# alibaba/TePDist

Hardware: AMD Instinct MI355X
Metric: tokens/sec (higher is better)
Workload: dtype bf16; 1 GPU; model=gpt2-345m, global_batch=64, seq_len=1024, parallelism=auto-planned-graph:dp1tp1pp1mesh[]micro1

## Files before the change

### tepdist_amd/ops/csrc/attention.hip

```cpp

#include <algorithm>
#include <stdexcept>

#include "common.h"
#include "kernels.h"
#include "lds_frag.h"

namespace tepdist {

namespace {

constexpr int NT = 256;
constexpr int QB = 128;
constexpr int KB = 64;

constexpr float kLog2e = 1.4426950408889634f;
DEV_INLINE float fast_exp(float x) {
  return __builtin_amdgcn_exp2f(x * kLog2e);
}

#define BAR_LDS()                                        \
  do {                                                   \
    asm volatile("s_waitcnt lgkmcnt(0)" ::: "memory");   \
    __builtin_amdgcn_s_barrier();                        \
  } while (0)

DEV_INLINE float warp16_max(float v) {
#pragma unroll
  for (int d = 1; d < 16; d <<= 1) v = fmaxf(v, __shfl_xor(v, d, 64));
  return v;
}

DEV_INLINE float warp16_sum(float v) {
#pragma unroll
  for (int d = 1; d < 16; d <<= 1) v += __shfl_xor(v, d, 64);
  return v;
}


constexpr int NTF = 512;
constexpr int QBF = 512;

template <int NQ>
DEV_INLINE int pair_row0(int q0, int wave, int hp) {
  return NQ == 4 ? q0 + 32 * (hp ? 15 - wave : wave) : q0 + 32 * wave;
}

template <int D, int NQ = (D == 64 ? 4 : 2)>
__launch_bounds__(NTF) __global__
void flash_fwd_kernel(const bf16_t* __restrict__ Q,
                      const bf16_t* __restrict__ K,
                      const bf16_t* __restrict__ V, bf16_t* __restrict__ O,
                      float* __restrict__ LSE, int S, int H, float scale,
                      bool causal, int64_t q_bs, int64_t q_hs, int64_t q_rs,
                      int64_t o_bs, int64_t o_hs, int64_t o_rs) {
  constexpr int DK = D / 32;
  constexpr int DF = D / 16;
  const int bh = blockIdx.y;
  const int b = bh / H, h = bh % H;
  const int q0 = blockIdx.x * (128 * NQ);
  const int wave = __builtin_amdgcn_readfirstlane(threadIdx.x >> 6);
  const int lane = threadIdx.x & 63;
  const int g = lane >> 4;

  const bf16_t* qp = Q + (int64_t)b * q_bs + (int64_t)h * q_hs;
  const bf16_t* kp = K + (int64_t)b * q_bs + (int64_t)h * q_hs;
  const bf16_t* vp = V + (int64_t)b * q_bs + (int64_t)h * q_hs;
  bf16_t* op = O + (int64_t)b * o_bs + (int64_t)h * o_hs;

  __shared__ __attribute__((aligned(16))) bf16_t smem[2 * 2 * KB * D];
  const int BUFSZ = 2 * KB * D;

  bf16x8 qf[NQ][DK];
#pragma unroll
  for (int nf = 0; nf < NQ; ++nf)
#pragma unroll
    for (int kk = 0; kk < DK; ++kk) {
      const int row = pair_row0<NQ>(q0, wave, nf >> 1) + (nf & 1) * 16 +
                      (lane & 15);
      bf16x8 v8 = {};
      if (row < S)
        v8 = *reinterpret_cast<const bf16x8*>(
            qp + (int64_t)row * q_rs + kk * 32 + 8 * g);
      qf[nf][kk] = v8;
    }

  const float sl2 = scale * kLog2e;
  f32x4 acc_o[DF][NQ] = {};
  float m_r[NQ], l_r[NQ];
#pragma unroll
  for (int i = 0; i < NQ; ++i) {
    m_r[i] = -3.0e38f;
    l_r[i] = 0.f;
  }

  constexpr int KUN = KB * D / 8 / NTF;
  bf16x8 krg[KUN], vrg[KUN];

  auto stage_load = [&](int kv0) {
#pragma unroll
    for (int u = 0; u < KUN; ++u) {
      const int idx = threadIdx.x + u * NTF;
      const int row = idx / (D / 8);
      const int c = (idx % (D / 8)) * 8;
      bf16x8 k8 = {}, v8 = {};
      if (kv0 + row < S) {
        k8 = *reinterpret_cast<const bf16x8*>(
            kp + (int64_t)(kv0 + row) * q_rs + c);
        v8 = *reinterpret_cast<const bf16x8*>(
            vp + (int64_t)(kv0 + row) * q_rs + c);
      }
      krg[u] = k8;
      vrg[u] = v8;
    }
  };
  auto stage_write = [&](int buf) {
    bf16_t* sK = smem + buf * BUFSZ;
    bf16_t* sV = sK + KB * D;
#pragma unroll
    for (int u = 0; u < KUN; ++u) {
      const int idx = threadIdx.x + u * NTF;
      const int row = idx / (D / 8);
      const int c = (idx % (D / 8)) * 8;
      *reinterpret_cast<bf16x8*>(sK + loff<D>(row, c)) = krg[u];
      *reinterpret_cast<bf16x8*>(sV + loff<D>(row, c)) = vrg[u];
    }
  };

  const int kv_end = causal ? min(S, q0 + 128 * NQ) : S;
  stage_load(0);
  stage_write(0);
  __syncthreads();
  int t = 0;
  for (int kv0 = 0; kv0 < kv_end; kv0 += KB, ++t) {
    const bf16_t* sK = smem + (t & 1) * BUFSZ;
    const bf16_t* sV = sK + KB * D;
    if (kv0 + KB < kv_end) stage_load(kv0 + KB);

    if (!causal || kv0 <= pair_row0<NQ>(q0, wave, NQ / 2 - 1) + 31) {
#pragma unroll
      for (int hp = 0; hp < NQ / 2; ++hp) {
        const int pq0 = pair_row0<NQ>(q0, wave, hp);
        if (causal && kv0 > pq0 + 31) continue;
        f32x4 st[4][2] = {};
        __builtin_amdgcn_s_setprio(1);
#pragma unroll
        for (int kk = 0; kk < DK; ++kk)
#pragma unroll
          for (int mi = 0; mi < 4; ++mi) {
            const bf16x8 kf = *reinterpret_cast<const bf16x8*>(
                sK + loff<D>((lane & 15) + 16 * mi, 8 * g + 32 * kk));
#pragma unroll
            for (int nf = 0; nf < 2; ++nf)
              st[mi][nf] = __builtin_amdgcn_mfma_f32_16x16x32_bf16(
                  kf, qf[2 * hp + nf][kk], st[mi][nf], 0, 0, 0);
          }
        __builtin_amdgcn_s_setprio(0);
        const bool inner = kv0 + KB <= pq0 && kv0 + KB <= S &&
                           pq0 + 32 <= S;
#pragma unroll
        for (int nf = 0; nf < 2; ++nf) {
          const int nfg = 2 * hp + nf;
          const int qg = pq0 + nf * 16 + (lane & 15);
          float tmax = -3.0e38f;
          if (inner) {
#pragma unroll
            for (int mi = 0; mi < 4; ++mi)
#pragma unroll
              for (int e = 0; e < 4; ++e)
                tmax = fmaxf(tmax, st[mi][nf][e]);
          } else {
#pragma unroll
            for (int mi = 0; mi < 4; ++mi)
#pragma unroll
              for (int e = 0; e < 4; ++e) {
                const int kg = kv0 + mi * 16 + 4 * g + e;
                const bool masked = (causal && kg > qg) || kg >= S ||
                                    qg >= S;
                const float sv = masked ? -3.0e38f : st[mi][nf][e];
                st[mi][nf][e] = sv;
                tmax = fmaxf(tmax, sv);
              }
          }
          tmax = fmaxf(tmax, __shfl_xor(tmax, 16, 64));
          tmax = fmaxf(tmax, __shfl_xor(tmax, 32, 64));
          const float mn = fmaxf(m_r[nfg], tmax * scale);
          const float alpha = fast_exp(m_r[nfg] - mn);
          m_r[nfg] = mn;
          const float nm2 = -mn * kLog2e;
          float rs = 0.f;
#pragma unroll
          for (int mi = 0; mi < 4; ++mi)
#pragma unroll
            for (int e = 0; e < 4; ++e) {
              const float p = __builtin_amdgcn_exp2f(
                  __builtin_fmaf(st[mi][nf][e], sl2, nm2));
              st[mi][nf][e] = p;
              rs += p;
            }
          rs += __shfl_xor(rs, 16, 64);
          rs += __shfl_xor(rs, 32, 64);
          l_r[nfg] = l_r[nfg] * alpha + rs;
#pragma unroll
          for (int df = 0; df < DF; ++df)
#pragma unroll
            for (int e = 0; e < 4; ++e) acc_o[df][nfg][e] *= alpha;
        }
        __builtin_amdgcn_s_setprio(1);
#pragma unroll
        for (int c = 0; c < KB / 32; ++c) {
          bf16x8 pb[2];
#pragma unroll
          for (int nf = 0; nf < 2; ++nf)
#pragma unroll
            for (int e = 0; e < 4; ++e) {
              pb[nf][e] = f2bf(st[2 * c][nf][e]);
              pb[nf][e + 4] = f2bf(st[2 * c + 1][nf][e]);
            }
#pragma unroll
          for (int df = 0; df < DF; ++df) {
            const bf16x8 vfr = tr_frag<D>(sV, c, df, lane);
#pragma unroll
            for (int nf = 0; nf < 2; ++nf)
              acc_o[df][2 * hp + nf] = __builtin_amdgcn_mfma_f32_16x16x32_bf16(
                  vfr, pb[nf], acc_o[df][2 * hp + nf], 0, 0, 0);
          }
        }
        __builtin_amdgcn_s_setprio(0);
      }
    }
    if (kv0 + KB < kv_end) stage_write((t + 1) & 1);
    BAR_LDS();
  }

#pragma unroll
  for (int nf = 0; nf < NQ; ++nf) {
    const int qg = pair_row0<NQ>(q0, wave, nf >> 1) + (nf & 1) * 16 +
                   (lane & 15);
    if (qg >= S) continue;
    const float lv = l_r[nf];
    const float inv = (lv > 0.f) ? 1.0f / lv : 0.f;
    if (g == 0)
      LSE[(int64_t)bh * S + qg] =
          (lv > 0.f) ? m_r[nf] + __logf(lv) : -3.0e38f;
#pragma unroll
    for (int df = 0; df < DF; ++df)
#pragma unroll
      for (int e = 0; e < 4; ++e)
        op[(int64_t)qg * o_rs + 16 * df + 4 * g + e] =
            f2bf(acc_o[df][nf][e] * inv);
  }
}

}

void attention_fwd_bf16(const void* q, const void* k, const void* v, void* o,
                        float* lse, int B, int H, int S, int D, float scale,
                        bool causal, int64_t q_bs, int64_t q_hs, int64_t q_rs,
                        int64_t o_bs, int64_t o_hs, int64_t o_rs,
                        hipStream_t stream) {
  dim3 block(NTF);
#define FWD_D(DD)                                                        \
  do {                                                                   \
    dim3 grid((S + (DD == 64 ? QBF : 256) - 1) / (DD == 64 ? QBF : 256), \
              B * H);                                                    \
    hipLaunchKernelGGL(flash_fwd_kernel<DD>, grid, block, 0, stream,     \
                       static_cast<const bf16_t*>(q),                    \
                       static_cast<const bf16_t*>(k),                    \
                       static_cast<const bf16_t*>(v),                    \
                       static_cast<bf16_t*>(o), lse, S, H, scale,        \
                       causal, q_bs, q_hs, q_rs, o_bs, o_hs, o_rs);      \
  } while (0)
  if (D == 64) FWD_D(64);
  else if (D == 128) FWD_D(128);
  else throw std::runtime_error("flash fwd: head dim must be 64 or 128");
#undef FWD_D
}

namespace {


template <int D>
__launch_bounds__(NT) __global__
void flash_bwd_delta_kernel(const bf16_t* __restrict__ dO,
                            const bf16_t* __restrict__ O,
                            float* __restrict__ delta, int64_t rows) {
  const int lane = threadIdx.x & 63;
  const int wid = threadIdx.x >> 6;
  const int64_t nw = (int64_t)gridDim.x * (NT / WAVE);
  for (int64_t r = (int64_t)blockIdx.x * (NT / WAVE) + wid; r < rows;
       r += nw) {
    float s = 0.f;
    for (int c = lane * 8; c < D; c += WAVE * 8) {
      const bf16x8 a = *reinterpret_cast<const bf16x8*>(dO + r * D + c);
      const bf16x8 b = *reinterpret_cast<const bf16x8*>(O + r * D + c);
#pragma unroll
      for (int e = 0; e < 8; ++e) s += bf2f(a[e]) * bf2f(b[e]);
    }
    s = wave_allreduce_sum(s);
    if (lane == 0) delta[r] = s;
  }
}

constexpr int NTA = 512;

template <int D, int KBA = (D == 64 ? 256 : 128)>
__launch_bounds__(NTA) __global__
void flash_bwd_kv_kernel(const bf16_t* __restrict__ Q,
                         const bf16_t* __restrict__ K,
                         const bf16_t* __restrict__ V,
                         const bf16_t* __restrict__ dO,
                         const float* __restrict__ LSE,
                         const float* __restrict__ DELTA,
                         bf16_t* __restrict__ dK, bf16_t* __restrict__ dV,
                         int S, int H, float scale, bool causal,
                         int64_t q_bs, int64_t q_hs, int64_t q_rs,
                         int64_t o_bs, int64_t o_hs, int64_t o_rs) {
  constexpr int DK = D / 32;
  constexpr int DF = D / 16;
  constexpr int QT = 64;
  constexpr int NSL = KBA / 128;
  const int bh = blockIdx.y;
  const int b = bh / H, h = bh % H;
  const int kv0 = blockIdx.x * KBA;
  const int wave = __builtin_amdgcn_readfirstlane(threadIdx.x >> 6);
  const int lane = threadIdx.x & 63;
  const int g = lane >> 4;

  const int64_t qoff = (int64_t)b * q_bs + (int64_t)h * q_hs;
  const int64_t ooff = (int64_t)b * o_bs + (int64_t)h * o_hs;
  const bf16_t* qp = Q + qoff;
  const bf16_t* kp = K + qoff;
  const bf16_t* vp = V + qoff;
  const bf16_t* dop = dO + ooff;

  __shared__ __attribute__((aligned(16))) bf16_t
      smem[KBA * D * 2 + QT * D * 2];
  bf16_t* sKb = smem;
  bf16_t* sVb = sKb + KBA * D;
  bf16_t* sQ = sVb + KBA * D;
  bf16_t* sdO = sQ + QT * D;
  __shared__ __attribute__((aligned(16))) float sNL2[QT], sDELTA[QT];
  const float sl2 = scale * kLog2e;

  {
    constexpr int UN = KBA * D / 8 / NTA;
#pragma unroll
    for (int u = 0; u < UN; ++u) {
      const int idx = threadIdx.x + u * NTA;
      const int row = idx / (D / 8);
      const int c = (idx % (D / 8)) * 8;
      bf16x8 kv8 = {}, vv8 = {};
      if (kv0 + row < S) {
        kv8 = *reinterpret_cast<const bf16x8*>(
            kp + (int64_t)(kv0 + row) * q_rs + c);
        vv8 = *reinterpret_cast<const bf16x8*>(
            vp + (int64_t)(kv0 + row) * q_rs + c);
      }
      *reinterpret_cast<bf16x8*>(sKb + loff<D>(row, c)) = kv8;
      *reinterpret_cast<bf16x8*>(sVb + loff<D>(row, c)) = vv8;
    }
  }
  __syncthreads();

  f32x4 acc_dkT[NSL][DF] = {};
  f32x4 acc_dvT[NSL][DF] = {};

  constexpr int QUN = QT * D / 8 / NTA;
  bf16x8 qn[QUN], don[QUN];
  float lse2[QT / NTA + 1], dl2[QT / NTA + 1];

  auto tile_load = [&](int q0) {
#pragma unroll
    for (int u = 0; u < QUN; ++u) {
      const int idx = threadIdx.x + u * NTA;
      const int row = idx / (D / 8);
      const int c = (idx % (D / 8)) * 8;
      bf16x8 a = {}, b2 = {};
      if (q0 + row < S) {
        a = *reinterpret_cast<const bf16x8*>(
            qp + (int64_t)(q0 + row) * q_rs + c);
        b2 = *reinterpret_cast<const bf16x8*>(
            dop + (int64_t)(q0 + row) * o_rs + c);
      }
      qn[u] = a;
      don[u] = b2;
    }
    for (int i = threadIdx.x, s2 = 0; i < QT; i += NTA, ++s2) {
      const int qg = q0 + i;
      const float l = (qg < S) ? LSE[(int64_t)bh * S + qg] : -3.0e38f;
      lse2[s2] = (l > -1.0e38f) ? -l * kLog2e : -3.0e38f;
      dl2[s2] = (qg < S) ? DELTA[(int64_t)bh * S + qg] : 0.f;
    }
  };
  auto tile_write = [&]() {
#pragma unroll
    for (int u = 0; u < QUN; ++u) {
      const int idx = threadIdx.x + u * NTA;
      const int row = idx / (D / 8);
      const int c = (idx % (D / 8)) * 8;
      *reinterpret_cast<bf16x8*>(sQ + loff<D>(row, c)) = qn[u];
      *reinterpret_cast<bf16x8*>(sdO + loff<D>(row, c)) = don[u];
    }
    for (int i = threadIdx.x, s2 = 0; i < QT; i += NTA, ++s2) {
      sNL2[i] = lse2[s2];
      sDELTA[i] = dl2[s2];
    }
  };

  const int q_start = causal ? (kv0 / QT) * QT : 0;
  tile_load(q_start);
  tile_write();
  __syncthreads();
  for (int q0 = q_start; q0 < S; q0 += QT) {
    if (q0 + QT < S) tile_load(q0 + QT);

#pragma unroll
    for (int sl = 0; sl < NSL; ++sl) {
      if (causal && kv0 + sl * 128 + wave * 16 > q0 + QT - 1) continue;
      f32x4 st[4] = {};
      f32x4 dpt[4] = {};
#pragma unroll
      for (int kk = 0; kk < DK; ++kk) {
        const bf16x8 kfr = *reinterpret_cast<const bf16x8*>(
            sKb + loff<D>(sl * 128 + wave * 16 + (lane & 15),
                          8 * g + 32 * kk));
        const bf16x8 vfr = *reinterpret_cast<const bf16x8*>(
            sVb + loff<D>(sl * 128 + wave * 16 + (lane & 15),
                          8 * g + 32 * kk));
#pragma unroll
        for (int mi = 0; mi < 4; ++mi) {
          const bf16x8 qa = *reinterpret_cast<const bf16x8*>(
              sQ + loff<D>(16 * mi + (lane & 15), 8 * g + 32 * kk));
          st[mi] = __builtin_amdgcn_mfma_f32_16x16x32_bf16(qa, kfr,
                                                           st[mi], 0, 0, 0);
          const bf16x8 da = *reinterpret_cast<const bf16x8*>(
              sdO + loff<D>(16 * mi + (lane & 15), 8 * g + 32 * kk));
          dpt[mi] = __builtin_amdgcn_mfma_f32_16x16x32_bf16(
              da, vfr, dpt[mi], 0, 0, 0);
        }
      }

      const int kvb = kv0 + sl * 128;
      const int kvg = kvb + wave * 16 + (lane & 15);
      const bool winner = (!causal || kvb + wave * 16 + 15 < q0) &&
                          q0 + QT <= S && kvb + 128 <= S;
      if (winner) {
        f32x4 nl2v[4], dlv[4];
#pragma unroll
        for (int mi = 0; mi < 4; ++mi) {
          nl2v[mi] = *reinterpret_cast<const f32x4*>(sNL2 + 16 * mi + 4 * g);
          dlv[mi] = *reinterpret_cast<const f32x4*>(sDELTA + 16 * mi + 4 * g);
        }
#pragma unroll
        for (int mi = 0; mi < 4; ++mi)
#pragma unroll
          for (int e = 0; e < 4; ++e) {
            const float pt = __builtin_amdgcn_exp2f(
                __builtin_fmaf(st[mi][e], sl2, nl2v[mi][e]));
            st[mi][e] = pt;
            dpt[mi][e] = pt * (dpt[mi][e] - dlv[mi][e]);
          }
      } else {
#pragma unroll
        for (int mi = 0; mi < 4; ++mi)
#pragma unroll
          for (int e = 0; e < 4; ++e) {
            const int qrow = 16 * mi + 4 * g + e;
            const int qg = q0 + qrow;
            const float nl2 = sNL2[qrow];
            const float dl = sDELTA[qrow];
            const bool valid = qg < S && kvg < S && (!causal || kvg <= qg) &&
                               nl2 > -1.0e38f;
            const float arg =
                valid ? __builtin_fmaf(st[mi][e], sl2, nl2) : -3.0e38f;
            const float pt = __builtin_amdgcn_exp2f(arg);
            st[mi][e] = pt;
            dpt[mi][e] = pt * (dpt[mi][e] - dl);
          }
      }

      __builtin_amdgcn_s_setprio(1);
#pragma unroll
      for (int c = 0; c < QT / 32; ++c) {
        bf16x8 pb, db;
#pragma unroll
        for (int e = 0; e < 4; ++e) {
          pb[e] = f2bf(st[2 * c][e]);
          pb[e + 4] = f2bf(st[2 * c + 1][e]);
          db[e] = f2bf(dpt[2 * c][e]);
          db[e + 4] = f2bf(dpt[2 * c + 1][e]);
        }
#pragma unroll
        for (int df = 0; df < DF; ++df) {
          const bf16x8 afr = tr_frag<D>(sdO, c, df, lane);
          const bf16x8 qfr = tr_frag<D>(sQ, c, df, lane);
          acc_dvT[sl][df] = __builtin_amdgcn_mfma_f32_16x16x32_bf16(
              afr, pb, acc_dvT[sl][df], 0, 0, 0);
          acc_dkT[sl][df] = __builtin_amdgcn_mfma_f32_16x16x32_bf16(
              qfr, db, acc_dkT[sl][df], 0, 0, 0);
        }
      }
      __builtin_amdgcn_s_setprio(0);
    }
    BAR_LDS();
    if (q0 + QT < S) {
      tile_write();
      BAR_LDS();
    }
  }

#pragma unroll
  for (int sl = 0; sl < NSL; ++sl) {
    const int kvg = kv0 + sl * 128 + wave * 16 + (lane & 15);
    if (kvg < S) {
#pragma unroll
      for (int df = 0; df < DF; ++df) {
        bf16x4 kv4, vv4;
#pragma unroll
        for (int e = 0; e < 4; ++e) {
          kv4[e] = f2bf(acc_dkT[sl][df][e] * scale);
          vv4[e] = f2bf(acc_dvT[sl][df][e]);
        }
        const int64_t off = qoff + (int64_t)kvg * q_rs + 16 * df + 4 * g;
        *reinterpret_cast<bf16x4*>(dK + off) = kv4;
        *reinterpret_cast<bf16x4*>(dV + off) = vv4;
      }
    }
  }
}

constexpr int NTB = 512;
constexpr int QBB = 256;

template <int D, int NQ = (D == 64 ? 4 : 2)>
__launch_bounds__(NTB) __global__
void flash_bwd_dq_kernel(const bf16_t* __restrict__ Q,
                         const bf16_t* __restrict__ K,
                         const bf16_t* __restrict__ V,
                         const bf16_t* __restrict__ dO,
                         const float* __restrict__ LSE,
                         const float* __restrict__ DELTA,
                         bf16_t* __restrict__ dQ, int S, int H, float scale,
                         bool causal, int64_t q_bs, int64_t q_hs,
                         int64_t q_rs, int64_t o_bs, int64_t o_hs,
                         int64_t o_rs) {
  constexpr int DK = D / 32;
  constexpr int DF = D / 16;
  const int bh = blockIdx.y;
  const int b = bh / H, h = bh % H;
  const int q0 = blockIdx.x * (128 * NQ);
  const int wave = __builtin_amdgcn_readfirstlane(threadIdx.x >> 6);
  const int lane = threadIdx.x & 63;
  const int g = lane >> 4;

  const int64_t qoff = (int64_t)b * q_bs + (int64_t)h * q_hs;
  const int64_t ooff = (int64_t)b * o_bs + (int64_t)h * o_hs;
  const bf16_t* qp = Q + qoff;
  const bf16_t* kp = K + qoff;
  const bf16_t* vp = V + qoff;
  const bf16_t* dop = dO + ooff;
  bf16_t* dqp = dQ + qoff;

  __shared__ __attribute__((aligned(16))) bf16_t smem[KB * D * 2];
  bf16_t* sK = smem;
  bf16_t* sV = smem + KB * D;

  const float sl2 = scale * kLog2e;
  bf16x8 qf[NQ][DK], dof[NQ][DK];
  float nl2_r[NQ], dl_r[NQ];
#pragma unroll
  for (int nf = 0; nf < NQ; ++nf) {
    const int row = pair_row0<NQ>(q0, wave, nf >> 1) + (nf & 1) * 16 +
                    (lane & 15);
    const float l = (row < S) ? LSE[(int64_t)bh * S + row] : -3.0e38f;
    nl2_r[nf] = (l > -1.0e38f) ? -l * kLog2e : -3.0e38f;
    dl_r[nf] = (row < S) ? DELTA[(int64_t)bh * S + row] : 0.f;
#pragma unroll
    for (int kk = 0; kk < DK; ++kk) {
      bf16x8 a = {}, b8 = {};
      if (row < S) {
        a = *reinterpret_cast<const bf16x8*>(
            qp + (int64_t)row * q_rs + kk * 32 + 8 * g);
        b8 = *reinterpret_cast<const bf16x8*>(
            dop + (int64_t)row * o_rs + kk * 32 + 8 * g);
      }
      qf[nf][kk] = a;
      dof[nf][kk] = b8;
    }
  }

  f32x4 acc_dq[DF][NQ] = {};

  constexpr int KUN = KB * D / 8 / NTB;
  bf16x8 krg[KUN], vrg[KUN];

  auto stage_load = [&](int kv0) {
#pragma unroll
    for (int u = 0; u < KUN; ++u) {
      const int idx = threadIdx.x + u * NTB;
      const int row = idx / (D / 8);
      const int c = (idx % (D / 8)) * 8;
      bf16x8 kv8 = {}, vv8 = {};
      if (kv0 + row < S) {
        kv8 = *reinterpret_cast<const bf16x8*>(
            kp + (int64_t)(kv0 + row) * q_rs + c);
        vv8 = *reinterpret_cast<const bf16x8*>(
            vp + (int64_t)(kv0 + row) * q_rs + c);
      }
      krg[u] = kv8;
      vrg[u] = vv8;
    }
  };
  auto stage_write = [&]() {
#pragma unroll
    for (int u = 0; u < KUN; ++u) {
      const int idx = threadIdx.x + u * NTB;
      const int row = idx / (D / 8);
      const int c = (idx % (D / 8)) * 8;
      *reinterpret_cast<bf16x8*>(sK + loff<D>(row, c)) = krg[u];
      *reinterpret_cast<bf16x8*>(sV + loff<D>(row, c)) = vrg[u];
    }
  };

  const int kv_end = causal ? min(S, q0 + 128 * NQ) : S;
  stage_load(0);
  stage_write();
  __syncthreads();
  for (int kv0 = 0; kv0 < kv_end; kv0 += KB) {
    if (kv0 + KB < kv_end) stage_load(kv0 + KB);

    if (!causal || kv0 <= pair_row0<NQ>(q0, wave, NQ / 2 - 1) + 31) {
#pragma unroll
     for (int hp = 0; hp < NQ / 2; ++hp) {
      const int pq0 = pair_row0<NQ>(q0, wave, hp);
      if (causal && kv0 > pq0 + 31) continue;
      const bool inner = kv0 + KB <= pq0 && kv0 + KB <= S && pq0 + 32 <= S;
      bf16x4 dsb[4][2];
#pragma unroll
      for (int mi = 0; mi < 4; ++mi) {
        f32x4 st[2] = {};
        f32x4 dpt[2] = {};
        __builtin_amdgcn_s_setprio(1);
#pragma unroll
        for (int kk = 0; kk < DK; ++kk) {
          const bf16x8 ka = *reinterpret_cast<const bf16x8*>(
              sK + loff<D>((lane & 15) + 16 * mi, 8 * g + 32 * kk));
          const bf16x8 va = *reinterpret_cast<const bf16x8*>(
              sV + loff<D>((lane & 15) + 16 * mi, 8 * g + 32 * kk));
#pragma unroll
          for (int nf = 0; nf < 2; ++nf) {
            st[nf] = __builtin_amdgcn_mfma_f32_16x16x32_bf16(
                ka, qf[2 * hp + nf][kk], st[nf], 0, 0, 0);
            dpt[nf] = __builtin_amdgcn_mfma_f32_16x16x32_bf16(
                va, dof[2 * hp + nf][kk], dpt[nf], 0, 0, 0);
          }
        }
        __builtin_amdgcn_s_setprio(0);
#pragma unroll
        for (int nf = 0; nf < 2; ++nf) {
          const int nfg = 2 * hp + nf;
          const int qg = pq0 + nf * 16 + (lane & 15);
          if (inner) {
#pragma unroll
            for (int e = 0; e < 4; ++e) {
              const float pt = __builtin_amdgcn_exp2f(
                  __builtin_fmaf(st[nf][e], sl2, nl2_r[nfg]));
              dsb[mi][nf][e] =
                  f2bf(pt * (dpt[nf][e] - dl_r[nfg]));
            }
          } else {
#pragma unroll
            for (int e = 0; e < 4; ++e) {
              const int kg = kv0 + 16 * mi + 4 * g + e;
              const bool valid = qg < S && kg < S &&
                                 (!causal || kg <= qg) &&
                                 nl2_r[nfg] > -1.0e38f;
              const float arg =
                  valid ? __builtin_fmaf(st[nf][e], sl2, nl2_r[nfg])
                        : -3.0e38f;
              const float pt = __builtin_amdgcn_exp2f(arg);
              dsb[mi][nf][e] =
                  f2bf(pt * (dpt[nf][e] - dl_r[nfg]));
            }
          }
        }
      }
      __builtin_amdgcn_s_setprio(1);
#pragma unroll
      for (int c = 0; c < KB / 32; ++c) {
        bf16x8 db[2];
#pragma unroll
        for (int nf = 0; nf < 2; ++nf)
#pragma unroll
          for (int e = 0; e < 4; ++e) {
            db[nf][e] = dsb[2 * c][nf][e];
            db[nf][e + 4] = dsb[2 * c + 1][nf][e];
          }
#pragma unroll
        for (int df = 0; df < DF; ++df) {
          const bf16x8 kfr = tr_frag<D>(sK, c, df, lane);
#pragma unroll
          for (int nf = 0; nf < 2; ++nf)
            acc_dq[df][2 * hp + nf] = __builtin_amdgcn_mfma_f32_16x16x32_bf16(
                kfr, db[nf], acc_dq[df][2 * hp + nf], 0, 0, 0);
        }
      }
      __builtin_amdgcn_s_setprio(0);
     }
    }
    BAR_LDS();
    if (kv0 + KB < kv_end) {
      stage_write();
      BAR_LDS();
    }
  }

#pragma unroll
  for (int nf = 0; nf < NQ; ++nf) {
    const int qg = pair_row0<NQ>(q0, wave, nf >> 1) + (nf & 1) * 16 +
                   (lane & 15);
    if (qg >= S) continue;
#pragma unroll
    for (int df = 0; df < DF; ++df) {
      bf16x4 v4;
#pragma unroll
      for (int e = 0; e < 4; ++e) v4[e] = f2bf(acc_dq[df][nf][e] * scale);
      *reinterpret_cast<bf16x4*>(
          dqp + (int64_t)qg * q_rs + 16 * df + 4 * g) = v4;
    }
  }
}


template <int D>
__global__ void flash_bwd_delta_strided_kernel(
    const bf16_t* __restrict__ dO, const bf16_t* __restrict__ O,
    float* __restrict__ delta, int H, int S, int64_t o_bs, int64_t o_hs,
    int64_t o_rs) {
  constexpr int LPR = D / 8;
  constexpr int RPW = WAVE / LPR;
  const int lane = threadIdx.x & 63;
  const int wid = threadIdx.x >> 6;
  const int sub = lane / LPR;
  const int c = (lane % LPR) * 8;
  const int64_t nr = (int64_t)gridDim.x * (NT / WAVE) * RPW;
  const int bh = blockIdx.y;
  const int b = bh / H, h = bh % H;
  const int64_t off = (int64_t)b * o_bs + (int64_t)h * o_hs;
  for (int64_t r0 = ((int64_t)blockIdx.x * (NT / WAVE) + wid) * RPW;
       r0 < S; r0 += nr) {
    const int64_t r = r0 + sub;
    float s = 0.f;
    if (r < S) {
      const bf16x8 a =
          *reinterpret_cast<const bf16x8*>(dO + off + r * o_rs + c);
      const bf16x8 bb =
          *reinterpret_cast<const bf16x8*>(O + off + r * o_rs + c);
#pragma unroll
      for (int e = 0; e < 8; ++e) s += bf2f(a[e]) * bf2f(bb[e]);
    }
#pragma unroll
    for (int d2 = 1; d2 < LPR; d2 <<= 1) s += __shfl_xor(s, d2, 64);
    if (r < S && (lane % LPR) == 0) delta[(int64_t)bh * S + r] = s;
  }
}

}



void attention_bwd_bf16(const void* q, const void* k, const void* v,
                        const void* o, const void* dout, const float* lse,
                        float* delta, void* dq, void* dk, void* dv,
                        int B, int H, int S, int D, float scale, bool causal,
                        int64_t q_bs, int64_t q_hs, int64_t q_rs,
                        int64_t o_bs, int64_t o_hs, int64_t o_rs,
                        hipStream_t stream) {
  dim3 block(NT);
#define BWD_D(DD)                                                            \
  do {                                                                       \
    dim3 dgrid((S / 4 + (NT / WAVE) - 1) / (NT / WAVE) > 256                 \
                   ? 256 : (S + 3) / 4, B * H);                              \
    hipLaunchKernelGGL(flash_bwd_delta_strided_kernel<DD>, dgrid, block, 0,  \
                       stream, static_cast<const bf16_t*>(dout),             \
                       static_cast<const bf16_t*>(o), delta, H, S, o_bs,     \
                       o_hs, o_rs);                                          \
    dim3 kgrid((S + (DD == 64 ? 255 : 127)) / (DD == 64 ? 256 : 128),       \
               B * H);                                                       \
    hipLaunchKernelGGL(flash_bwd_kv_kernel<DD>, kgrid, dim3(512), 0, stream, \
                       static_cast<const bf16_t*>(q),                        \
                       static_cast<const bf16_t*>(k),                        \
                       static_cast<const bf16_t*>(v),                        \
                       static_cast<const bf16_t*>(dout), lse, delta,         \
                       static_cast<bf16_t*>(dk), static_cast<bf16_t*>(dv),   \
                       S, H, scale, causal, q_bs, q_hs, q_rs, o_bs, o_hs,    \
                       o_rs);                                                \
    dim3 qgrid((S + (DD == 64 ? 511 : 255)) / (DD == 64 ? 512 : 256),       \
               B * H);                                                       \
    hipLaunchKernelGGL(flash_bwd_dq_kernel<DD>, qgrid, dim3(NTB), 0, stream, \
                       static_cast<const bf16_t*>(q),                        \
                       static_cast<const bf16_t*>(k),                        \
                       static_cast<const bf16_t*>(v),                        \
                       static_cast<const bf16_t*>(dout), lse, delta,         \
                       static_cast<bf16_t*>(dq), S, H, scale, causal, q_bs,  \
                       q_hs, q_rs, o_bs, o_hs, o_rs);                        \
  } while (0)
  if (D == 64) BWD_D(64);
  else if (D == 128) BWD_D(128);
  else throw std::runtime_error("flash bwd: head dim must be 64 or 128");
#undef BWD_D
}
}
```

Measured before the change: 338,300 tokens/s.

## Specialize attention tiles by mask mode, double-buffer dQ K/V, defer row-sum reduction

The forward kernel's per-tile work is split into templated score, softmax and PV lambdas, dispatched by compile-time mask mode (interior vs boundary). The boundary mask is simplified to a single per-lane limit compare. Cross-lane max uses permlane16/32 swaps instead of shuffles, and the row-sum reduction is moved out of the loop to once at the epilogue. The dQ backward kernel gets double-buffered K/V shared memory so one barrier per tile suffices, and its score MFMAs are software-pipelined one block ahead of the dS computation. This trades more LDS and registers (which may reduce occupancy) for fewer barriers and less masking and shuffle overhead.

Measured after the change: 344,100 tokens/s (median of 6 runs). 1.7% higher.

```diff
diff --git a/tepdist_amd/ops/csrc/attention.hip b/tepdist_amd/ops/csrc/attention.hip
--- a/tepdist_amd/ops/csrc/attention.hip
+++ b/tepdist_amd/ops/csrc/attention.hip
@@ -1,6 +1,7 @@
 
 #include <algorithm>
 #include <stdexcept>
+#include <type_traits>
 
 #include "common.h"
 #include "kernels.h"
@@ -24,6 +25,29 @@
     asm volatile("s_waitcnt lgkmcnt(0)" ::: "memory");   \
     __builtin_amdgcn_s_barrier();                        \
   } while (0)
+
+#define PAIR_FENCE() asm volatile("" ::: "memory")
+
+template <int V>
+using ic = std::integral_constant<int, V>;
+
+DEV_INLINE float quad_max(float v) {
+  const unsigned u = __float_as_uint(v);
+  const auto a = __builtin_amdgcn_permlane16_swap(u, u, false, false);
+  const unsigned w = __float_as_uint(
+      fmaxf(__uint_as_float(a[0]), __uint_as_float(a[1])));
+  const auto b = __builtin_amdgcn_permlane32_swap(w, w, false, false);
+  return fmaxf(__uint_as_float(b[0]), __uint_as_float(b[1]));
+}
+
+DEV_INLINE float quad_sum(float v) {
+  const unsigned u = __float_as_uint(v);
+  const auto a = __builtin_amdgcn_permlane16_swap(u, u, false, false);
+  const unsigned w =
+      __float_as_uint(__uint_as_float(a[0]) + __uint_as_float(a[1]));
+  const auto b = __builtin_amdgcn_permlane32_swap(w, w, false, false);
+  return __uint_as_float(b[0]) + __uint_as_float(b[1]);
+}
 
 DEV_INLINE float warp16_max(float v) {
 #pragma unroll
@@ -127,6 +151,106 @@
     }
   };
 
+  auto scores = [&](auto hp_c, const bf16_t* sK, f32x4 (&st)[4][2]) {
+    constexpr int hp = decltype(hp_c)::value;
+    __builtin_amdgcn_s_setprio(1);
+#pragma unroll
+    for (int kk = 0; kk < DK; ++kk)
+#pragma unroll
+      for (int mi = 0; mi < 4; ++mi) {
+        const bf16x8 kf = *reinterpret_cast<const bf16x8*>(
+            sK + loff<D>((lane & 15) + 16 * mi, 8 * g + 32 * kk));
+#pragma unroll
+        for (int nf = 0; nf < 2; ++nf)
+          st[mi][nf] = __builtin_amdgcn_mfma_f32_16x16x32_bf16(
+              kf, qf[2 * hp + nf][kk], st[mi][nf], 0, 0, 0);
+      }
+    __builtin_amdgcn_s_setprio(0);
+  };
+  auto softmax = [&](auto hp_c, auto mode_c, f32x4 (&st)[4][2], int kv0,
+                     int pq0, bool interior) {
+    constexpr int hp = decltype(hp_c)::value;
+    constexpr int mode = decltype(mode_c)::value;
+#pragma unroll
+    for (int nf = 0; nf < 2; ++nf) {
+      const int nfg = 2 * hp + nf;
+      float tmax = -3.0e38f;
+      if (mode == 1 || (mode == 2 && !interior)) {
+        const int qg = pq0 + nf * 16 + (lane & 15);
+        int lim = S - 1 - kv0 - 4 * g;
+        if (causal) lim = min(lim, qg - kv0 - 4 * g);
+        if (qg >= S) lim = -1;
+#pragma unroll
+        for (int mi = 0; mi < 4; ++mi)
+#pragma unroll
+          for (int e = 0; e < 4; ++e) {
+            const bool masked = 16 * mi + e > lim;
+            const float sv = masked ? -3.0e38f : st[mi][nf][e];
+            st[mi][nf][e] = sv;
+            tmax = fmaxf(tmax, sv);
+          }
+      } else {
+#pragma unroll
+        for (int mi = 0; mi < 4; ++mi)
+#pragma unroll
+          for (int e = 0; e < 4; ++e) tmax = fmaxf(tmax, st[mi][nf][e]);
+      }
+      tmax = quad_max(tmax);
+      const float mn = fmaxf(m_r[nfg], tmax * scale);
+      const float alpha = fast_exp(m_r[nfg] - mn);
+      m_r[nfg] = mn;
+      const float nm2 = -mn * kLog2e;
+      float rs = 0.f;
+#pragma unroll
+      for (int mi = 0; mi < 4; ++mi)
+#pragma unroll
+        for (int e = 0; e < 4; ++e) {
+          const float p = __builtin_amdgcn_exp2f(
+              __builtin_fmaf(st[mi][nf][e], sl2, nm2));
+          st[mi][nf][e] = p;
+          rs += p;
+        }
+      l_r[nfg] = l_r[nfg] * alpha + rs;
+#pragma unroll
+      for (int df = 0; df < DF; ++df)
+#pragma unroll
+        for (int e = 0; e < 4; ++e) acc_o[df][nfg][e] *= alpha;
+    }
+  };
+  auto pv = [&](auto hp_c, const bf16_t* sV, f32x4 (&st)[4][2]) {
+    constexpr int hp = decltype(hp_c)::value;
+    __builtin_amdgcn_s_setprio(1);
+#pragma unroll
+    for (int c = 0; c < KB / 32; ++c) {
+      bf16x8 pb[2];
+#pragma unroll
+      for (int nf = 0; nf < 2; ++nf)
+#pragma unroll
+        for (int e = 0; e < 4; ++e) {
+          pb[nf][e] = f2bf(st[2 * c][nf][e]);
+          pb[nf][e + 4] = f2bf(st[2 * c + 1][nf][e]);
+        }
+#pragma unroll
+      for (int df = 0; df < DF; ++df) {
+        const bf16x8 vfr = tr_frag<D>(sV, c, df, lane);
+#pragma unroll
+        for (int nf = 0; nf < 2; ++nf)
+          acc_o[df][2 * hp + nf] = __builtin_amdgcn_mfma_f32_16x16x32_bf16(
+              vfr, pb[nf], acc_o[df][2 * hp + nf], 0, 0, 0);
+      }
+    }
+    __builtin_amdgcn_s_setprio(0);
+  };
+  auto pair_tile = [&](auto hp_c, auto mode_c, const bf16_t* sK,
+                       const bf16_t* sV, int kv0, int pq0,
+                       bool interior = false) {
+    PAIR_FENCE();
+    f32x4 st[4][2] = {};
+    scores(hp_c, sK, st);
+    softmax(hp_c, mode_c, st, kv0, pq0, interior);
+    pv(hp_c, sV, st);
+  };
+
   const int kv_end = causal ? min(S, q0 + 128 * NQ) : S;
   stage_load(0);
   stage_write(0);
@@ -137,97 +261,28 @@
     const bf16_t* sV = sK + KB * D;
     if (kv0 + KB < kv_end) stage_load(kv0 + KB);
 
-    if (!causal || kv0 <= pair_row0<NQ>(q0, wave, NQ / 2 - 1) + 31) {
-#pragma unroll
-      for (int hp = 0; hp < NQ / 2; ++hp) {
-        const int pq0 = pair_row0<NQ>(q0, wave, hp);
-        if (causal && kv0 > pq0 + 31) continue;
-        f32x4 st[4][2] = {};
-        __builtin_amdgcn_s_setprio(1);
-#pragma unroll
-        for (int kk = 0; kk < DK; ++kk)
-#pragma unroll
-          for (int mi = 0; mi < 4; ++mi) {
-            const bf16x8 kf = *reinterpret_cast<const bf16x8*>(
-                sK + loff<D>((lane & 15) + 16 * mi, 8 * g + 32 * kk));
-#pragma unroll
-            for (int nf = 0; nf < 2; ++nf)
-              st[mi][nf] = __builtin_amdgcn_mfma_f32_16x16x32_bf16(
-                  kf, qf[2 * hp + nf][kk], st[mi][nf], 0, 0, 0);
-          }
-        __builtin_amdgcn_s_setprio(0);
-        const bool inner = kv0 + KB <= pq0 && kv0 + KB <= S &&
-                           pq0 + 32 <= S;
-#pragma unroll
-        for (int nf = 0; nf < 2; ++nf) {
-          const int nfg = 2 * hp + nf;
-          const int qg = pq0 + nf * 16 + (lane & 15);
-          float tmax = -3.0e38f;
-          if (inner) {
-#pragma unroll
-            for (int mi = 0; mi < 4; ++mi)
-#pragma unroll
-              for (int e = 0; e < 4; ++e)
-                tmax = fmaxf(tmax, st[mi][nf][e]);
-          } else {
-#pragma unroll
-            for (int mi = 0; mi < 4; ++mi)
-#pragma unroll
-              for (int e = 0; e < 4; ++e) {
-                const int kg = kv0 + mi * 16 + 4 * g + e;
-                const bool masked = (causal && kg > qg) || kg >= S ||
-                                    qg >= S;
-                const float sv = masked ? -3.0e38f : st[mi][nf][e];
-                st[mi][nf][e] = sv;
-                tmax = fmaxf(tmax, sv);
-              }
-          }
-          tmax = fmaxf(tmax, __shfl_xor(tmax, 16, 64));
-          tmax = fmaxf(tmax, __shfl_xor(tmax, 32, 64));
-          const float mn = fmaxf(m_r[nfg], tmax * scale);
-          const float alpha = fast_exp(m_r[nfg] - mn);
-          m_r[nfg] = mn;
-          const float nm2 = -mn * kLog2e;
-          float rs = 0.f;
-#pragma unroll
-          for (int mi = 0; mi < 4; ++mi)
-#pragma unroll
-            for (int e = 0; e < 4; ++e) {
-              const float p = __builtin_amdgcn_exp2f(
-                  __builtin_fmaf(st[mi][nf][e], sl2, nm2));
-              st[mi][nf][e] = p;
-              rs += p;
-            }
-          rs += __shfl_xor(rs, 16, 64);
-          rs += __shfl_xor(rs, 32, 64);
-          l_r[nfg] = l_r[nfg] * alpha + rs;
-#pragma unroll
-          for (int df = 0; df < DF; ++df)
-#pragma unroll
-            for (int e = 0; e < 4; ++e) acc_o[df][nfg][e] *= alpha;
-        }
-        __builtin_amdgcn_s_setprio(1);
-#pragma unroll
-        for (int c = 0; c < KB / 32; ++c) {
-          bf16x8 pb[2];
-#pragma unroll
-          for (int nf = 0; nf < 2; ++nf)
-#pragma unroll
-            for (int e = 0; e < 4; ++e) {
-              pb[nf][e] = f2bf(st[2 * c][nf][e]);
-              pb[nf][e + 4] = f2bf(st[2 * c + 1][nf][e]);
-            }
-#pragma unroll
-          for (int df = 0; df < DF; ++df) {
-            const bf16x8 vfr = tr_frag<D>(sV, c, df, lane);
-#pragma unroll
-            for (int nf = 0; nf < 2; ++nf)
-              acc_o[df][2 * hp + nf] = __builtin_amdgcn_mfma_f32_16x16x32_bf16(
-                  vfr, pb[nf], acc_o[df][2 * hp + nf], 0, 0, 0);
-          }
-        }
-        __builtin_amdgcn_s_setprio(0);
-      }
+    const int pq_lo = pair_row0<NQ>(q0, wave, 0);
+    const int pq_hi = pair_row0<NQ>(q0, wave, NQ / 2 - 1);
+    const bool tile_in = kv0 + KB <= S;
+    const bool in_lo = tile_in && (!causal || kv0 + KB <= pq_lo) &&
+                       pq_lo + 32 <= S;
+    const bool in_hi = tile_in && (!causal || kv0 + KB <= pq_hi) &&
+                       pq_hi + 32 <= S;
+    if constexpr (NQ == 4) {
+      if (in_lo && in_hi) {
+        pair_tile(ic<0>{}, ic<0>{}, sK, sV, kv0, pq_lo);
+        pair_tile(ic<1>{}, ic<0>{}, sK, sV, kv0, pq_hi);
+      } else {
+        if (!causal || kv0 <= pq_lo + 31)
+          pair_tile(ic<0>{}, ic<1>{}, sK, sV, kv0, pq_lo);
+        if (!causal || kv0 <= pq_hi + 31) {
+          if (in_hi) pair_tile(ic<1>{}, ic<0>{}, sK, sV, kv0, pq_hi);
+          else pair_tile(ic<1>{}, ic<1>{}, sK, sV, kv0, pq_hi);
+        }
+      }
+    } else {
+      if (!causal || kv0 <= pq_hi + 31)
+        pair_tile(ic<0>{}, ic<2>{}, sK, sV, kv0, pq_hi, in_hi);
     }
     if (kv0 + KB < kv_end) stage_write((t + 1) & 1);
     BAR_LDS();
@@ -237,8 +292,8 @@
   for (int nf = 0; nf < NQ; ++nf) {
     const int qg = pair_row0<NQ>(q0, wave, nf >> 1) + (nf & 1) * 16 +
                    (lane & 15);
+    const float lv = quad_sum(l_r[nf]);
     if (qg >= S) continue;
-    const float lv = l_r[nf];
     const float inv = (lv > 0.f) ? 1.0f / lv : 0.f;
     if (g == 0)
       LSE[(int64_t)bh * S + qg] =
@@ -562,9 +617,10 @@
   const bf16_t* dop = dO + ooff;
   bf16_t* dqp = dQ + qoff;
 
-  __shared__ __attribute__((aligned(16))) bf16_t smem[KB * D * 2];
-  bf16_t* sK = smem;
-  bf16_t* sV = smem + KB * D;
+  __shared__ __attribute__((aligned(16))) bf16_t smem[2 * KB * D * 2];
+  const int BUFSZ = 2 * KB * D;
+  const bf16_t* sK = smem;
+  const bf16_t* sV = smem + KB * D;
 
   const float sl2 = scale * kLog2e;
   bf16x8 qf[NQ][DK], dof[NQ][DK];
@@ -612,114 +668,156 @@
       vrg[u] = vv8;
     }
   };
-  auto stage_write = [&]() {
+  auto stage_write = [&](int buf) {
+    bf16_t* wK = smem + buf * BUFSZ;
+    bf16_t* wV = wK + KB * D;
 #pragma unroll
     for (int u = 0; u < KUN; ++u) {
       const int idx = threadIdx.x + u * NTB;
       const int row = idx / (D / 8);
       const int c = (idx % (D / 8)) * 8;
-      *reinterpret_cast<bf16x8*>(sK + loff<D>(row, c)) = krg[u];
-      *reinterpret_cast<bf16x8*>(sV + loff<D>(row, c)) = vrg[u];
-    }
+      *reinterpret_cast<bf16x8*>(wK + loff<D>(row, c)) = krg[u];
+      *reinterpret_cast<bf16x8*>(wV + loff<D>(row, c)) = vrg[u];
+    }
+  };
+
+  auto score_block = [&](auto hp_c, int mi, f32x4 (&st)[2],
+                         f32x4 (&dpt)[2]) {
+    constexpr int hp = decltype(hp_c)::value;
+    __builtin_amdgcn_s_setprio(1);
+#pragma unroll
+    for (int kk = 0; kk < DK; ++kk) {
+      const bf16x8 ka = *reinterpret_cast<const bf16x8*>(
+          sK + loff<D>((lane & 15) + 16 * mi, 8 * g + 32 * kk));
+      const bf16x8 va = *reinterpret_cast<const bf16x8*>(
+          sV + loff<D>((lane & 15) + 16 * mi, 8 * g + 32 * kk));
+#pragma unroll
+      for (int nf = 0; nf < 2; ++nf) {
+        st[nf] = __builtin_amdgcn_mfma_f32_16x16x32_bf16(
+            ka, qf[2 * hp + nf][kk], kk ? st[nf] : f32x4{}, 0, 0, 0);
+        dpt[nf] = __builtin_amdgcn_mfma_f32_16x16x32_bf16(
+            va, dof[2 * hp + nf][kk], kk ? dpt[nf] : f32x4{}, 0, 0, 0);
+      }
+    }
+    __builtin_amdgcn_s_setprio(0);
+  };
+  auto ds_block = [&](auto hp_c, auto mode_c, int mi, const f32x4 (&st)[2],
+                      const f32x4 (&dpt)[2], bf16x4 (&dsb)[2], int kv0,
+                      int pq0, bool interior) {
+    constexpr int hp = decltype(hp_c)::value;
+    constexpr int mode = decltype(mode_c)::value;
+#pragma unroll
+    for (int nf = 0; nf < 2; ++nf) {
+      const int nfg = 2 * hp + nf;
+      if (mode == 0 || (mode == 2 && interior)) {
+#pragma unroll
+        for (int e = 0; e < 4; ++e) {
+          const float pt = __builtin_amdgcn_exp2f(
+              __builtin_fmaf(st[nf][e], sl2, nl2_r[nfg]));
+          dsb[nf][e] = f2bf(pt * (dpt[nf][e] - dl_r[nfg]));
+        }
+      } else {
+        const int qg = pq0 + nf * 16 + (lane & 15);
+        int lim = S - 1 - kv0 - 4 * g;
+        if (causal) lim = min(lim, qg - kv0 - 4 * g);
+        if (qg >= S || !(nl2_r[nfg] > -1.0e38f)) lim = -1;
+#pragma unroll
+        for (int e = 0; e < 4; ++e) {
+          const bool valid = 16 * mi + e <= lim;
+          const float arg =
+              valid ? __builtin_fmaf(st[nf][e], sl2, nl2_r[nfg]) : -3.0e38f;
+          const float pt = __builtin_amdgcn_exp2f(arg);
+          dsb[nf][e] = f2bf(pt * (dpt[nf][e] - dl_r[nfg]));
+        }
+      }
+    }
+  };
+  auto pair_tile = [&](auto hp_c, auto mode_c, int kv0, int pq0,
+                       bool interior = false) {
+    constexpr int hp = decltype(hp_c)::value;
+    PAIR_FENCE();
+    bf16x4 dsb[4][2];
+    if constexpr (NQ == 4) {
+      f32x4 st[2][2], dpt[2][2];
+      score_block(hp_c, 0, st[0], dpt[0]);
+#pragma unroll
+      for (int mi = 0; mi < 4; ++mi) {
+        if (mi + 1 < 4)
+          score_block(hp_c, mi + 1, st[(mi + 1) & 1], dpt[(mi + 1) & 1]);
+        ds_block(hp_c, mode_c, mi, st[mi & 1], dpt[mi & 1], dsb[mi], kv0,
+                 pq0, interior);
+      }
+    } else {
+#pragma unroll
+      for (int mi = 0; mi < 4; ++mi) {
+        f32x4 st[2], dpt[2];
+        score_block(hp_c, mi, st, dpt);
+        ds_block(hp_c, mode_c, mi, st, dpt, dsb[mi], kv0, pq0, interior);
+      }
+    }
+    __builtin_amdgcn_s_setprio(1);
+#pragma unroll
+    for (int c = 0; c < KB / 32; ++c) {
+      bf16x8 db[2];
+#pragma unroll
+      for (int nf = 0; nf < 2; ++nf)
+#pragma unroll
+        for (int e = 0; e < 4; ++e) {
+          db[nf][e] = dsb[2 * c][nf][e];
+          db[nf][e + 4] = dsb[2 * c + 1][nf][e];
+        }
+#pragma unroll
+      for (int df = 0; df < DF; ++df) {
+        const bf16x8 kfr = tr_frag<D>(sK, c, df, lane);
+#pragma unroll
+        for (int nf = 0; nf < 2; ++nf)
+          acc_dq[df][2 * hp + nf] = __builtin_amdgcn_mfma_f32_16x16x32_bf16(
+              kfr, db[nf], acc_dq[df][2 * hp + nf], 0, 0, 0);
+      }
+    }
+    __builtin_amdgcn_s_setprio(0);
   };
 
   const int kv_end = causal ? min(S, q0 + 128 * NQ) : S;
   stage_load(0);
-  stage_write();
+  stage_write(0);
   __syncthreads();
-  for (int kv0 = 0; kv0 < kv_end; kv0 += KB) {
+  int t = 0;
+  for (int kv0 = 0; kv0 < kv_end; kv0 += KB, ++t) {
+    sK = smem + (t & 1) * BUFSZ;
+    sV = sK + KB * D;
     if (kv0 + KB < kv_end) stage_load(kv0 + KB);
 
-    if (!causal || kv0 <= pair_row0<NQ>(q0, wave, NQ / 2 - 1) + 31) {
-#pragma unroll
-     for (int hp = 0; hp < NQ / 2; ++hp) {
-      const int pq0 = pair_row0<NQ>(q0, wave, hp);
-      if (causal && kv0 > pq0 + 31) continue;
-      const bool inner = kv0 + KB <= pq0 && kv0 + KB <= S && pq0 + 32 <= S;
-      bf16x4 dsb[4][2];
-#pragma unroll
-      for (int mi = 0; mi < 4; ++mi) {
-        f32x4 st[2] = {};
-        f32x4 dpt[2] = {};
-        __builtin_amdgcn_s_setprio(1);
-#pragma unroll
-        for (int kk = 0; kk < DK; ++kk) {
-          const bf16x8 ka = *reinterpret_cast<const bf16x8*>(
-              sK + loff<D>((lane & 15) + 16 * mi, 8 * g + 32 * kk));
-          const bf16x8 va = *reinterpret_cast<const bf16x8*>(
-              sV + loff<D>((lane & 15) + 16 * mi, 8 * g + 32 * kk));
-#pragma unroll
-          for (int nf = 0; nf < 2; ++nf) {
-            st[nf] = __builtin_amdgcn_mfma_f32_16x16x32_bf16(
-                ka, qf[2 * hp + nf][kk], st[nf], 0, 0, 0);
-            dpt[nf] = __builtin_amdgcn_mfma_f32_16x16x32_bf16(
-                va, dof[2 * hp + nf][kk], dpt[nf], 0, 0, 0);
-          }
-        }
-        __builtin_amdgcn_s_setprio(0);
-#pragma unroll
-        for (int nf = 0; nf < 2; ++nf) {
-          const int nfg = 2 * hp + nf;
-          const int qg = pq0 + nf * 16 + (lane & 15);
-          if (inner) {
-#pragma unroll
-            for (int e = 0; e < 4; ++e) {
-              const float pt = __builtin_amdgcn_exp2f(
-                  __builtin_fmaf(st[nf][e], sl2, nl2_r[nfg]));
-              dsb[mi][nf][e] =
-                  f2bf(pt * (dpt[nf][e] - dl_r[nfg]));
-            }
-          } else {
-#pragma unroll
-            for (int e = 0; e < 4; ++e) {
-              const int kg = kv0 + 16 * mi + 4 * g + e;
-              const bool valid = qg < S && kg < S &&
-                                 (!causal || kg <= qg) &&
-                                 nl2_r[nfg] > -1.0e38f;
-              const float arg =
-                  valid ? __builtin_fmaf(st[nf][e], sl2, nl2_r[nfg])
-                        : -3.0e38f;
-              const float pt = __builtin_amdgcn_exp2f(arg);
-              dsb[mi][nf][e] =
-                  f2bf(pt * (dpt[nf][e] - dl_r[nfg]));
-            }
-          }
-        }
-      }
-      __builtin_amdgcn_s_setprio(1);
-#pragma unroll
-      for (int c = 0; c < KB / 32; ++c) {
-        bf16x8 db[2];
-#pragma unroll
-        for (int nf = 0; nf < 2; ++nf)
-#pragma unroll
-          for (int e = 0; e < 4; ++e) {
-            db[nf][e] = dsb[2 * c][nf][e];
-            db[nf][e + 4] = dsb[2 * c + 1][nf][e];
-          }
-#pragma unroll
-        for (int df = 0; df < DF; ++df) {
-          const bf16x8 kfr = tr_frag<D>(sK, c, df, lane);
-#pragma unroll
-          for (int nf = 0; nf < 2; ++nf)
-            acc_dq[df][2 * hp + nf] = __builtin_amdgcn_mfma_f32_16x16x32_bf16(
-                kfr, db[nf], acc_dq[df][2 * hp + nf], 0, 0, 0);
-        }
-      }
-      __builtin_amdgcn_s_setprio(0);
-     }
-    }
+    const int pq_lo = pair_row0<NQ>(q0, wave, 0);
+    const int pq_hi = pair_row0<NQ>(q0, wave, NQ / 2 - 1);
+    const bool tile_in = kv0 + KB <= S;
+    const bool in_lo = tile_in && (!causal || kv0 + KB <= pq_lo) &&
+                       pq_lo + 32 <= S;
+    const bool in_hi = tile_in && (!causal || kv0 + KB <= pq_hi) &&
+                       pq_hi + 32 <= S;
+    if constexpr (NQ == 4) {
+      if (!causal || kv0 <= pq_lo + 31) {
+        if (in_lo) pair_tile(ic<0>{}, ic<0>{}, kv0, pq_lo);
+        else pair_tile(ic<0>{}, ic<1>{}, kv0, pq_lo);
+      }
+      if (!causal || kv0 <= pq_hi + 31) {
+        if (in_hi) pair_tile(ic<1>{}, ic<0>{}, kv0, pq_hi);
+        else pair_tile(ic<1>{}, ic<1>{}, kv0, pq_hi);
+      }
+    } else {
+      if (!causal || kv0 <= pq_hi + 31)
+        pair_tile(ic<0>{}, ic<2>{}, kv0, pq_hi, in_hi);
+    }
+    if (kv0 + KB < kv_end) stage_write((t + 1) & 1);
     BAR_LDS();
-    if (kv0 + KB < kv_end) {
-      stage_write();
-      BAR_LDS();
-    }
-  }
-
+  }
+
+  int lane_e = lane;
+  asm volatile("" : "+v"(lane_e));
 #pragma unroll
   for (int nf = 0; nf < NQ; ++nf) {
     const int qg = pair_row0<NQ>(q0, wave, nf >> 1) + (nf & 1) * 16 +
-                   (lane & 15);
+                   (lane_e & 15);
     if (qg >= S) continue;
 #pragma unroll
     for (int df = 0; df < DF; ++df) {
@@ -727,7 +825,7 @@
 #pragma unroll
       for (int e = 0; e < 4; ++e) v4[e] = f2bf(acc_dq[df][nf][e] * scale);
       *reinterpret_cast<bf16x4*>(
-          dqp + (int64_t)qg * q_rs + 16 * df + 4 * g) = v4;
+          dqp + (int64_t)qg * q_rs + 16 * df + 4 * (lane_e >> 4)) = v4;
     }
   }
 }
```
